# WHU-USI3DV/GAGS

Measured on AMD Instinct MI355X. Metric: feature-raster fwd+bwd views/s, higher is better.
Workload: dtype f32

## Files before the change

### gags_amd/_lib.py

```python
import ctypes
import os
import subprocess

import torch

_HERE = os.path.dirname(os.path.abspath(__file__))
CSRC = os.path.join(_HERE, "csrc")
LIB_PATH = os.path.join(CSRC, "libgags_hip.so")

_vp, _i32, _i64, _f32, _f64 = ctypes.c_void_p, ctypes.c_int, ctypes.c_int64, ctypes.c_float, ctypes.c_double

SIGNATURES = {
    "gags_abi_version": (_i32, []),
    "gags_strerror": (ctypes.c_char_p, [_i32]),
    "gags_device_count": (_i32, []),
    "gags_project_fwd": (_i32, [_i32, _vp, _vp, _vp, _vp, _vp, _i32, _i32, _f32, _f32, _f32, _f32,
                                _vp, _vp, _vp, _vp, _vp, _vp]),
    "gags_project_fwd_raw": (_i32, [_i32, _vp, _vp, _vp, _vp, _f32, _vp, _vp, _i32, _i32, _f32, _f32, _f32, _f32,
                                    _vp, _vp, _vp, _vp, _vp, _vp, _vp, _vp, _vp, _vp]),
    "gags_project_bwd_raw": (_i32, [_i32, _vp, _vp, _vp, _vp, _f32, _vp, _vp, _i32, _i32, _f32, _vp, _vp, _vp, _vp, _vp,
                                    _vp, _vp, _vp, _vp, _vp]),
    "gags_scan_scratch_bytes": (_i64, [_i32]),
    "gags_cumsum_i32": (_i32, [_i32, _vp, _vp, _vp, _vp, _i64, _vp]),
    "gags_cumsum_gather_i32": (_i32, [_i32, _vp, _vp, _vp, _vp, _vp, _i64, _vp]),
# ... 55 lines not shown
    "gags_sam_clip_feature": (_i32, [_i32, _i32, _i32, _i32, _i32, _i32, _vp, _vp, _vp, _vp, _vp, _vp]),
    "gags_sam_clip_feature_bwd_scale": (_i32, [_i32, _i32, _i32, _i32, _i32, _i32, _vp, _vp, _vp, _vp, _vp]),
    "gags_distill_l1_map_fwd": (_i32, [_i32, _i32, _i32, _i32, _i32, _i32, _vp, _vp, _vp, _vp, _vp, _vp, _i32, _vp]),
    "gags_distill_l1_map_bwd": (_i32, [_i32, _i32, _i32, _i32, _i32, _i32, _vp, _vp, _vp, _vp, _vp, _vp, _vp, _i32, _vp]),
    "gags_decoder_head_distill_fwd": (_i32, [_i32, _i32, _i32, _i32, _i32, _i32, _i32, _vp, _vp, _vp, _vp, _vp, _vp, _vp]),
    "gags_decoder_head_distill_bwd": (_i32, [_i32, _i32, _i32, _i32, _i32, _i32, _i32, _vp, _vp, _vp, _vp, _vp, _vp, _vp, _vp]),
    "gags_decoder_head_distill_bwd_f32": (_i32, [_i32, _i32, _i32, _i32, _i32, _i32, _i32, _vp, _vp, _vp, _vp, _vp, _vp, _vp, _vp]),
    "gags_decoder_pack_input": (_i32, [_i64, _i32, _i32, _vp, _vp, _vp]),
    "gags_decoder_pack_layer": (_i32, [_i32, _i32, _vp, _vp, _vp, _vp, _vp, _vp, _vp, _vp]),
    "gags_decoder_pack_layers": (_i32, [_i32, _vp, _vp, _vp, _vp, _vp, _vp, _vp, _vp, _vp, _vp]),
    "gags_decoder_layer": (_i32, [_i64, _i32, _i32, _vp, _vp, _vp, _vp, _i32, _vp, _vp, _vp, _vp, _vp, _vp]),
    "gags_decoder_wgrad_scratch_bytes": (_i64, [_i64, _i32, _i32]),
    "gags_decoder_wgrad": (_i32, [_i64, _i32, _i32, _vp, _vp, _vp, _vp, _vp, _vp, _i64, _vp]),
    "gags_decoder_wgrad_out": (_i32, [_i64, _i32, _i32, _vp, _vp, _vp, _vp, _vp, _i32, _i32, _vp, _vp, _i64, _vp]),
    "gags_decoder_head_bwd": (_i32, [_i64, _i32, _i32, _i32, _vp, _vp, _vp, _i32, _vp]),
    "gags_decoder_unpack_grad": (_i32, [_i64, _i32, _i32, _vp, _vp, _vp]),
    "gags_decoder_head": (_i32, [_i64, _i32, _i32, _i32, _vp, _vp, _i32, _vp]),
    "gags_decoder_fwd_fused": (_i32, [_i64, _i32, _i32, _vp, _vp, _vp, _vp, _vp, _vp, _vp]),
    "gags_decoder_bwd_fused": (_i32, [_i64, _i32, _i32, _vp, _vp, _vp, _vp, _vp, _vp]),
    "gags_decoder_bwd_fused_scaled": (_i32, [_i64, _i32, _i32, _vp, _vp, _vp, _vp, _vp, _vp, _vp]),
    "gags_scale_decoder_fwd_fused": (_i32, [_i64, _i32, _vp, _vp, _vp, _vp, _vp, _vp, _vp]),
    "gags_scale_decoder_fwd_fused_head": (_i32, [_i64, _i32, _vp, _vp, _vp, _vp, _vp, _vp, _vp, _vp]),
    "gags_softmax_head_bwd_y": (_i32, [_i64, _i32, _i32, _vp, _vp, _vp, _vp]),
    "gags_scale_decoder_bwd_fused": (_i32, [_i64, _vp, _vp, _vp, _vp, _vp]),
    "gags_decoder_layer_exact": (_i32, [_i64, _i32, _i32, _vp, _vp, _i32, _vp, _vp, _i32, _vp, _vp, _vp, _vp, _i32, _vp]),
    "gags_decoder_layer_split": (_i32, [_i64, _i32, _i32, _vp, _vp, _i32, _vp, _vp, _i32, _vp, _vp, _vp, _vp, _i32, _i32, _vp]),
    "gags_decoder_wgrad_split": (_i32, [_i64, _i32, _i32, _vp, _i32, _vp, _vp, _i32, _vp, _vp, _vp, _i64, _i32, _vp]),
    "gags_decoder_wgrad_exact_scratch_bytes": (_i64, [_i64, _i32, _i32]),
    "gags_decoder_wgrad_exact": (_i32, [_i64, _i32, _i32, _vp, _i32, _vp, _vp, _i32, _vp, _vp, _vp, _i64, _vp]),
    "gags_decoder_head_bwd_exact": (_i32, [_i64, _i32, _i32, _i32, _vp, _vp, _i32, _vp, _i32, _vp]),
    **{name + "_h16": None for name in ("gags_decoder_pack_layer", "gags_decoder_pack_layers", "gags_decoder_pack_input", "gags_decoder_layer", "gags_decoder_head",
                                        "gags_decoder_wgrad_scratch_bytes", "gags_decoder_wgrad", "gags_decoder_wgrad_out",
                                        "gags_decoder_head_bwd",
                                        "gags_decoder_unpack_grad", "gags_decoder_fwd_fused", "gags_decoder_bwd_fused", "gags_decoder_bwd_fused_scaled",
                                        "gags_scale_decoder_fwd_fused", "gags_scale_decoder_bwd_fused", "gags_scale_decoder_fwd_fused_head",
                                        "gags_softmax_head_bwd_y")},
    "gags_pow2_scale": (_i32, [_vp, _f32, _f32, _vp, _vp]),
    "gags_decoder_head_distill_bwd_h16": (_i32, [_i32, _i32, _i32, _i32, _i32, _i32, _i32, _vp, _vp, _vp, _vp, _vp, _vp, _vp, _vp, _vp]),
    "gags_relevancy": (_i32, [_i64, _i32, _i32, _i32, _vp, _vp, _vp, _vp, _vp]),
    "gags_relevancy_activate_scratch_bytes": (_i64, [_i32, _i32, _i32]),
    "gags_relevancy_activate": (_i32, [_i32, _i32, _i32, _vp, _f32, _i32, _i32, _vp, _vp, _vp, _vp, _vp, _vp, _vp, _i64, _vp]),
    "gags_point_relevancy_mask_scratch_bytes": (_i64, [_i32, _i64]),
    "gags_point_relevancy_mask": (_i32, [_i32, _i64, _vp, _f32, _vp, _vp, _vp, _i64, _vp]),
    "gags_point_mask_smooth_scratch_bytes": (_i64, [_i32, _i64]),
    "gags_point_mask_smooth": (_i32, [_i32, _i64, _vp, _vp, _f64, _i32, _vp, _vp, _vp, _i64, _vp]),
    "gags_depthsample_scratch_bytes": (_i64, [_i64, _i32, _i32, _i32]),
    "gags_depthsample_map": (_i32, [_i64, _i32, _i32, _i32, _vp, _vp, _vp, _vp, _f32, _i32, _vp, _vp, _vp, _vp, _i64, _vp]),
    "gags_depthsample_scatter": (_i32, [_i64, _i32, _i32, _i32, _vp, _vp, _vp, _vp, _f32, _i32, _vp, _vp, _vp, _i64, _vp]),
    "gags_photometric_partials": (_i64, [_i32, _i32, _i32]),
    "gags_photometric_fwd": (_i32, [_i32, _i32, _i32, _i32, _vp, _i64, _i64, _i64, _vp, _i64, _i64, _i64, _vp, _f64, _f64, _f64,
                                    _i32, _vp, _vp, _vp, _vp, _vp, _vp, _vp]),
    "gags_photometric_bwd": (_i32, [_i32, _i32, _i32, _i32, _vp, _i64, _i64, _i64, _vp, _i64, _i64, _i64, _vp, _vp, _vp, _vp,
                                    _i64, _i64, _i64, _vp]),
    "gags_densify_stats": (_i32, [_i32, _vp, _vp, _vp, _vp, _f32, _f32, _vp, _vp, _vp, _vp]),
    "gags_densify_decide": (_i32, [_i32, _vp, _vp, _vp, _vp, _f32, _f32, _f32, _f32, _f32, _i32, _vp, _vp]),
    "gags_densify_plan": (_i32, [_i32, _vp, _vp, _vp, _i64, _vp, _vp, _vp, _vp]),
    "gags_densify_gather": (_i32, [_i64, _vp, _vp, _i32, _vp, _vp]),
    "gags_densify_children": (_i32, [_i64, _i64, _i32, _vp, _vp, _vp, _vp, _vp, _vp, _i64, _vp, _vp, _vp]),
    "gags_reset_opacity": (_i32, [_i64, _vp, _vp, _vp, _vp]),
    "gags_knn3_dist2_scratch_bytes": (_i64, [_i64]),
    "gags_knn3_dist2": (_i32, [_i64, _vp, _vp, _vp, _i64, _vp]),
    "gags_masks_max_count": (_i32, []),
    "gags_masks_pair_chunk_words": (_i32, []),
    "gags_masks_pack": (_i32, [_i32, _i64, _vp, _vp, _vp, _vp]),
    "gags_masks_pairs": (_i32, [_i32, _i64, _vp, _vp, _vp]),
    "gags_masks_colmax": (_i32, [_i32, _vp, _vp, _vp, _vp, _vp]),
    "gags_masks_paint": (_i32, [_i32, _i64, _vp, _i32, _vp, _i32, _vp, _vp]),
    "gags_masks_nms_scratch_bytes": (_i64, [_i32, _i64]),
    "gags_masks_nms_colmax": (_i32, [_i32, _i64, _vp, _vp, _vp, _vp, _vp, _i64, _vp]),
}

for _name in [k for k, v in SIGNATURES.items() if v is None]:
    SIGNATURES[_name] = SIGNATURES[_name[:-4]]

GAGS_BWD_COLORS_ONLY = 1
GAGS_FWD_NO_MFMA = 2
GAGS_FWD_ONLY_WEIGHTS, GAGS_FWD_ONLY_FEATURES = 512, 1024
GAGS_RECS_BY_GAUSSIAN = 256
GAGS_BWD_ATOMIC = 4
GAGS_FEAT_F16 = 32
GAGS_BWD_F32MFMA = 64
GAGS_BWD_BLOCKWAVES = 4096
GAGS_BWD_EXACT_WEIGHTS = 8192
GAGS_BWD_F16SPLIT = 0
GAGS_FWD_F16MFMA = 128
GAGS_FWD_F16MFMA_C = 64
GAGS_FWD_EXACT = 2048
GAGS_FWD_FUSED = 8
GAGS_STAGE_ALL, GAGS_STAGE_ROWS, GAGS_STAGE_SORT, GAGS_STAGE_REDUCE, GAGS_STAGE_MASK = 0, 1, 2, 3, 15
GAGS_STAGED_F32MFMA, GAGS_STAGED_OUT_F16, GAGS_STAGED_PREZEROED = 32, 64, 128
GAGS_STAGED_RANGE_SCRATCH, GAGS_STAGED_BLOCKWAVES, GAGS_STAGED_EXACT_WEIGHTS = 256, 512, 1024
GAGS_KIND_KEEP, GAGS_KIND_CLONE, GAGS_KIND_CHILD_A, GAGS_KIND_CHILD_B = 0, 1, 2, 3
GAGS_GATHER_MAX_DESC, GAGS_GATHER_COPY, GAGS_GATHER_MOMENT = 24, 0, 1


class GatherDesc(ctypes.Structure):
    _fields_ = [("in_", _vp), ("out", _vp), ("row_floats", ctypes.c_int32), ("mode", ctypes.c_int32)]


GAGS_GEOM_F32MFMA = 32

_lib = None


class GagsLibraryError(RuntimeError):
    pass


def build(verbose=False):
    out = None if verbose else subprocess.DEVNULL
    subprocess.check_call(["make", "-C", CSRC, "-j8", "libgags_hip.so"], stdout=out)
    return LIB_PATH


def load():
    global _lib
    if _lib is not None:
        return _lib
    if not os.path.exists(LIB_PATH):
        raise GagsLibraryError(
            f"{LIB_PATH} is missing: build it with `python -c 'import __graft_entry__ as g; g.build()'` "
            "or `make -C gags_amd/csrc`.  gags_amd has no CPU / PyTorch fallback.")
    try:
        lib = ctypes.CDLL(LIB_PATH)
    except OSError as e:
        raise GagsLibraryError(f"cannot load {LIB_PATH}: {e}") from e
    for name, (res, args) in SIGNATURES.items():
        try:
            fn = getattr(lib, name)
        except AttributeError as e:
            raise GagsLibraryError(f"{LIB_PATH} does not export {name}") from e
        fn.restype = res
        fn.argtypes = args
    _lib = lib
    return lib


def check(code, what):
    if code != 0:
        msg = load().gags_strerror(code)
        raise RuntimeError(f"{what} failed: {msg.decode() if msg else code} ({code})")


def ptr(t):
    return None if t is None else ctypes.c_void_p(t.data_ptr())
```

### gags_amd/csrc/launch.h

```cpp
#pragma once
#include "common.h"

inline int64_t al256(int64_t x) { return (x + 255) / 256 * 256; }

struct GagsTiles {
    int w, h, n;
};
inline GagsTiles gags_tiles(int width, int height)
{
    const int w = (width + GAGS_TILE - 1) / GAGS_TILE, h = (height + GAGS_TILE - 1) / GAGS_TILE;
    return {w, h, w * h};
}

constexpr int GAGS_MAX_DEVICES = 16;
template <int N>
inline bool gags_raise_dynamic_lds(bool (&raised)[GAGS_MAX_DEVICES], const void *const (&kernels)[N], int bytes)
{
    int dev = 0;
    if (hipGetDevice(&dev) != hipSuccess || dev < 0) return false;
    if (dev < GAGS_MAX_DEVICES && raised[dev]) return true;
    for (const void *k : kernels)
        if (hipFuncSetAttribute(k, hipFuncAttributeMaxDynamicSharedMemorySize, bytes) != hipSuccess) return false;
    if (dev < GAGS_MAX_DEVICES) raised[dev] = true;
    return true;
}

int64_t gags_sort_u32_scratch_bytes(int64_t n);
int gags_sort_pairs_u32(int64_t n, int nbits, const uint32_t *keys_in, const int32_t *vals_in, uint32_t *keys_out,
                        int32_t *vals_out, void *scratch, int64_t scratch_bytes, hipStream_t st);
int64_t gags_sort_u64_scratch_bytes(int64_t n);
int gags_sort_pairs_u64(int64_t n, int first_bit, int nbits, const uint64_t *keys_in, const int32_t *vals_in,
                        uint64_t *keys_out, int32_t *vals_out, void *scratch, int64_t scratch_bytes, hipStream_t st);

int gags_raster_fwd_valu(int d, int width, int height, const float *means2d, const float *conics,
                         const float *opacities, const float *colors, const float *backgrounds,
                         const int32_t *offsets, const int32_t *flat, int n_isects, float *out, float *alphas,
                         int32_t *last_ids, hipStream_t st);
int gags_raster_bwd_valu(int d, int width, int height, const float *means2d, const float *conics,
                         const float *opacities, const float *colors, const float *backgrounds,
                         const int32_t *offsets, const int32_t *flat, int n_isects, const float *alphas,
                         const int32_t *last_ids, const float *v_out, const float *v_alpha, float *v_colors,
                         float *v_opac, float *v_m2d, float *v_con, bool geom, hipStream_t st);

int gags_pack_isects_launch(int n, int n_isects, const int32_t *flat, const float *means2d, const float *conics,
                            const float *opacities, const int32_t *radii, void *grec, void *packed, hipStream_t st);
int gags_raster_weights_launch(int width, int height, int n_gauss, const void *packed, int by_gauss, const int32_t *offsets,
                               const int32_t *flat, int n_isects, float *wt, int32_t *gid_s, int32_t *sidx_s,
                               int32_t *hit, int32_t *blk_rows, float *Tbuf, float *alphas, int32_t *last_ids,
                               hipStream_t st, const float *colors16 = nullptr, const float *backgrounds = nullptr,
                               float *render_colors = nullptr);
int gags_list_need_launch(int width, int height, int n_gauss, const void *packed, int by_gauss, const int32_t *offsets,
                          const int32_t *flat, int n_isects, int32_t *need, hipStream_t st);
int gags_trim_offsets_launch(int n_tiles, const int32_t *cum, int32_t *off_new, hipStream_t st);
int gags_trim_gather_launch(int n_tiles, const int32_t *off_old, const int32_t *off_new, const int32_t *flat_in, int32_t *flat_out,
                            hipStream_t st);
int gags_trim_last_ids_launch(int width, int height, const int32_t *off_old, const int32_t *off_new, const float *alphas,
                              int32_t *last_ids, hipStream_t st);

int gags_raster_fwd_feat_launch(int d, int width, int height, int n_gauss, const float *colors, int colors_f16, int exact,
                                const float *backgrounds, const int32_t *offsets, int n_isects,
                                const int32_t *blk_rows, const float *wt, const int32_t *gid_s, const float *Tbuf,
                                float *out, hipStream_t st);
int gags_raster_fwd_fused_launch(int d, int width, int height, const void *packed, const float *colors,
                                 const float *backgrounds, const int32_t *offsets, const int32_t *flat, int n_isects,
                                 float *out, float *alphas, int32_t *last_ids, int by_gauss, hipStream_t st);

int64_t gags_bwd_staged_scratch_bytes_impl(int64_t rows, int n_gauss, int d);
int gags_raster_bwd_staged_launch(int d, int width, int height, int n_gauss, const int32_t *offsets, int n_isects,
                                  const float *v_out, const int32_t *blk_rows, const int32_t *trow, int64_t rows,
                                  const float *wt, const int32_t *gid_s, const int32_t *trow_s, void *scratch,
                                  int64_t scratch_bytes, float *v_colors, int stage_flags, int ch_begin, int ch_count,
                                  const int32_t *rows_dev, const int32_t *wire_pos, float *wire, const uint8_t *keep_prev,
                                  uint8_t *keep_cur, hipStream_t st);
int gags_bwd_slot_rows_launch(int width, int height, int n_isects, const int32_t *offsets, const int32_t *blk_rows,
                              const int32_t *sidx_s, const int32_t *trow, int32_t *trow_s, hipStream_t st);

int gags_rows_group_launch(int64_t rows, int n_gauss, const int32_t *rows_dev, uint32_t *key, int32_t *idx, uint32_t *key_s,
                           int32_t *idx_s, int32_t *seg, void *sort_scratch, int64_t sort_scratch_bytes, hipStream_t st);
int gags_rows_reduce_launch(int n_gauss, int d, int ch_begin, int ch_count, const int32_t *seg, const int32_t *idx_s,
                            const float *prow, int pitch, void *out, bool out_f16, hipStream_t st, int sparse = 0,
                            const int32_t *wire_pos = nullptr, float *wire = nullptr, const uint8_t *keep_prev = nullptr,
                            uint8_t *keep_cur = nullptr);

int64_t gags_raster_bwd_geom_scratch_bytes_impl(int64_t n_isects, int width, int height, int n_gauss, int d, int64_t n_rows);
int gags_raster_bwd_geom_launch(int d, int n_gauss, int width, int height, const float *colors, const float *backgrounds,
                                const int32_t *offsets, int n_isects, const void *packed, const float *v_out,
                                const float *v_alphas, const int32_t *blk_rows, const float *wt, const int32_t *gid_s,
                                const int32_t *sidx_s, const float *Tbuf, void *scratch, int64_t scratch_bytes, float *v_geo,
                                int by_gauss, const int32_t *row_base, int64_t n_rows, const int32_t *hit,
                                const int32_t *flatten_ids, int f32mfma, hipStream_t st);
int gags_blended_mask_launch(int n_isects, const int32_t *hit, const int32_t *flatten_ids, unsigned char *mask, hipStream_t st);

int gags_raster_bwd_atomic_launch(int d, int width, int height, const void *packed, const int32_t *offsets,
                                  const int32_t *flat, int n_isects, const float *v_out, float *v_colors,
                                  int by_gauss, hipStream_t st);
```

### gags_amd/csrc/raster_bwd_rows.hip

```cpp
#include <cstdlib>
#include "raster_mfma_common.h"
#include "launch.h"

using namespace gags_mfma;

namespace {

constexpr int CMAX = 64;

template <int NBR>
__global__ __launch_bounds__(256, (NBR == 4 ? 2 : (NBR == 2 ? 3 : 4))) void raster_bwd_rows(
    int d, int width, int height, int tile_w, int n_tiles, int ch_base, int n_slices,
    const float *__restrict__ v_render_colors, const int32_t *__restrict__ offsets, int n_isects,
    const int32_t *__restrict__ blk_rows, const int32_t *__restrict__ trow, const float *__restrict__ wt,
    const int32_t *__restrict__ gid_s, const int32_t *__restrict__ trow_s, float *__restrict__ prow, int prow_pitch,
    uint32_t *__restrict__ row_key, int32_t *__restrict__ row_idx, int rows_cap)
{
    constexpr int CW = 32 * NBR;
    constexpr int C4 = CW / 4;
    __shared__ __attribute__((aligned(16))) float stage[4][32][CW];
    __shared__ __attribute__((aligned(4))) uint8_t pos[2][CMAX][4];
    __shared__ int cand[2][4];
    __shared__ __attribute__((aligned(16))) float zrow[CW];

// ... 401 lines not shown
    L.seg = o; o += al256(((int64_t)n_gauss + 2) * 4);
    L.sort = o; o += al256(gags_sort_u32_scratch_bytes(rows));
    L.prow = o; o += al256(rows * (int64_t)d * 4);
    L.total = o;
    return L;
}

}

int64_t gags_bwd_staged_scratch_bytes_impl(int64_t rows, int n_gauss, int d)
{
    return staged_layout(rows > 0 ? rows : 1, n_gauss, d).total;
}

int gags_bwd_slot_rows_launch(int width, int height, int n_isects, const int32_t *offsets, const int32_t *blk_rows,
                              const int32_t *sidx_s, const int32_t *trow, int32_t *trow_s, hipStream_t st)
{
    GAGS_CLEAR_ERR();
    const int n_tiles = gags_tiles(width, height).n;
    hipLaunchKernelGGL(slot_rows_kernel, dim3(n_tiles * GAGS_BLOCKS_PER_TILE), dim3(64), 0, st, n_tiles, n_isects, offsets, blk_rows, sidx_s, trow, trow_s);
    GAGS_CHECK_LAUNCH();
    return GAGS_OK;
}

static bool rows_scale_per_block()
{
    static const bool v = [] { const char *e = getenv("GAGS_BWD_ROWSCALE"); return e && e[0] == '1'; }();
    return v;
}

int gags_raster_bwd_staged_launch(int d, int width, int height, int n_gauss, const int32_t *offsets, int n_isects,
                                  const float *v_out, const int32_t *blk_rows, const int32_t *trow, int64_t rows,
                                  const float *wt, const int32_t *gid_s, const int32_t *trow_s, void *scratch,
                                  int64_t scratch_bytes, float *v_colors, int stage_flags, int ch_begin, int ch_count,
                                  const int32_t *rows_dev, const int32_t *wire_pos, float *wire, const uint8_t *keep_prev,
                                  uint8_t *keep_cur, hipStream_t st)
{
    GAGS_CLEAR_ERR();
    const int stage = stage_flags & GAGS_STAGE_MASK;
    if (!gags_mfma_width(d) || d > 1024) return 1;
    const bool sA = stage == GAGS_STAGE_ALL || stage == GAGS_STAGE_ROWS, sS = stage == GAGS_STAGE_ALL || stage == GAGS_STAGE_SORT,
               sR = stage == GAGS_STAGE_ALL || stage == GAGS_STAGE_REDUCE;
    const GagsTiles T = gags_tiles(width, height);
    if (ch_count <= 0 || ch_begin < 0 || ch_begin + ch_count > d || ch_begin % 32 != 0 ||
        (ch_count % 32 != 0 && ch_begin + ch_count != d))
        return GAGS_EINVAL;
    const bool narrow = (stage_flags & GAGS_STAGED_RANGE_SCRATCH) != 0;
    const int pp = narrow ? ((ch_count + 3) & ~3) : d;
    const StagedLayout L = staged_layout(rows > 0 ? rows : 1, n_gauss, pp);
    if (scratch_bytes < L.total) return GAGS_ESCRATCH;
    char *sb = (char *)scratch;
    uint32_t *key = (uint32_t *)(sb + L.key), *key_s = (uint32_t *)(sb + L.key_s);
    int32_t *idx = (int32_t *)(sb + L.idx), *idx_s = (int32_t *)(sb + L.idx_s), *seg = (int32_t *)(sb + L.seg);
    float *prow = (float *)(sb + L.prow) - (narrow ? ch_begin : 0);
    if (rows > 0 && sA) {
#define GAGS_ROWS_LAUNCH(KERNEL, CH0, NSL)                                                                           \
    hipLaunchKernelGGL(KERNEL, dim3(T.n * (NSL)), dim3(256), 0, st, d, width, height, T.w, T.n, (CH0), (NSL),           \
                       v_out, offsets, n_isects, blk_rows, trow, wt, gid_s, trow_s, prow, pp, key, idx, (int)rows)
        int c = ch_begin;
        const int ce = ch_begin + ch_count;
        if (ce - c >= 128) {
            const int nsl = (ce - c) / 128;
            if (stage_flags & GAGS_STAGED_F32MFMA) GAGS_ROWS_LAUNCH(raster_bwd_rows<4>, c, nsl);
            else if (stage_flags & GAGS_STAGED_BLOCKWAVES) GAGS_ROWS_LAUNCH(raster_bwd_rows_f16, c, nsl);
            else if (stage_flags & GAGS_STAGED_EXACT_WEIGHTS) GAGS_ROWS_LAUNCH((raster_bwd_rows_cw<3, 5>), c, nsl);
            else if (rows_scale_per_block()) GAGS_ROWS_LAUNCH((raster_bwd_rows_cw<2, 3>), c, nsl);
            else GAGS_ROWS_LAUNCH((raster_bwd_rows_cw<2, 3, true>), c, nsl);
            c += 128 * nsl;
        }
        if (ce - c >= 64) {
            GAGS_ROWS_LAUNCH(raster_bwd_rows<2>, c, 1);
            c += 64;
        }
        if (ce - c > 0) GAGS_ROWS_LAUNCH(raster_bwd_rows<1>, c, (ce - c + 31) / 32);
#undef GAGS_ROWS_LAUNCH
    }
    if (sS) {
        const int rc = gags_rows_group_launch(rows, n_gauss, rows_dev, key, idx, key_s, idx_s, seg, sb + L.sort, L.prow - L.sort, st);
        if (rc != GAGS_OK) return rc;
    }
    if (sR) {
        const bool half = (stage_flags & GAGS_STAGED_OUT_F16) != 0;
        const int sparse = (stage_flags & GAGS_STAGED_PREZEROED) ? 1 : 0;
        const int rc = gags_rows_reduce_launch(n_gauss, d, ch_begin, ch_count, seg, idx_s, prow, pp, v_colors, half, st, sparse, wire_pos,
                                               wire, keep_prev, keep_cur);
        if (rc != GAGS_OK) return rc;
    }
    GAGS_CHECK_LAUNCH();
    return GAGS_OK;
}
```

### gags_amd/csrc/rows_reduce.hip

```cpp
#include <hip/hip_fp16.h>
#include "launch.h"

namespace {

__global__ __launch_bounds__(256) void row_tail_kernel(int64_t cap, const int32_t *__restrict__ total, int n_gauss,
                                                       uint32_t *__restrict__ row_key, int32_t *__restrict__ row_idx)
{
    const int64_t i = (int64_t)blockIdx.x * 256 + threadIdx.x;
    if (i >= cap || i < (int64_t)total[0]) return;
    row_key[i] = (uint32_t)n_gauss;
    row_idx[i] = 0;
}

__global__ __launch_bounds__(256) void seg_offsets_kernel(int n, const uint32_t *__restrict__ sorted_keys, int n_keys,
                                                          int32_t *__restrict__ seg)
{
    const int i = blockIdx.x * 256 + threadIdx.x;
    if (i >= n) return;
    const int cur = min((int)sorted_keys[i], n_keys);
    if (i == 0) {
        for (int g = 0; g <= cur; ++g) seg[g] = 0;
    } else {
        const int prev = min((int)sorted_keys[i - 1], n_keys);
        for (int g = prev + 1; g <= cur; ++g) seg[g] = i;
    }
    if (i == n - 1)
        for (int g = cur + 1; g <= n_keys; ++g) seg[g] = n;
}

__global__ void seg_fill_kernel(int n_keys, int32_t *__restrict__ seg)
{
    const int g = blockIdx.x * 256 + threadIdx.x;
    if (g <= n_keys) seg[g] = 0;
}

constexpr int REDUCE_ITER = 8;
template <bool HALF, int VW>
__global__ __launch_bounds__(256) void reduce_rows_kernel(int n_gauss, int d, int ch_begin, int ch_count,
                                                          const int32_t *__restrict__ seg,
                                                          const int32_t *__restrict__ sorted_rows,
                                                          const float *__restrict__ prow, int prow_pitch,
                                                          void *__restrict__ v_colors_, int sparse,
                                                          const int32_t *__restrict__ wire_pos, float *__restrict__ wire,
                                                          const uint8_t *__restrict__ keep_prev, uint8_t *__restrict__ keep_cur,
                                                          int tail)
{
    const int lpg = ch_count / VW;
    const int gpb = 256 / lpg;
    const int gl = threadIdx.x / lpg;
    const int cl = ch_begin + (threadIdx.x % lpg) * VW;
    if (gl >= gpb) return;
    for (int it = 0; it < REDUCE_ITER; ++it) {
    const int g = (blockIdx.x * REDUCE_ITER + it) * gpb + gl;
    if (g >= n_gauss) return;
        const int b = seg[g], e = seg[g + 1];
        const bool has = b != e;
        bool write_grad = sparse ? has : true;
        const bool on_wire = wire && wire_pos[g] >= 0;
        if (keep_cur) {
            if (threadIdx.x % lpg == 0) keep_cur[g] = (has || on_wire) ? 1 : 0;
            write_grad = has || keep_prev[g] != 0;
        }
        if (!write_grad && !on_wire) continue;
        const bool skip_grad = !write_grad;
        if constexpr (VW == 1) {
            float acc = 0.f;
            for (int i = b; i < e; ++i) acc += prow[(size_t)sorted_rows[i] * prow_pitch + cl];
            if (!skip_grad) {
                if constexpr (HALF) reinterpret_cast<__half *>(v_colors_)[(size_t)g * d + cl] = __float2half_rn(acc);
                else reinterpret_cast<float *>(v_colors_)[(size_t)g * d + cl] = acc;
            }
            if (wire) {
                const int q = wire_pos[g];
                if (q >= 0) wire[(size_t)q * ch_count + (cl - ch_begin)] = acc;
            }
        } else {
            float4 acc = make_float4(0.f, 0.f, 0.f, 0.f);
            const int tl = threadIdx.x % lpg;
            const bool has_tail = tl < tail;
            const int ct = ch_begin + ch_count + (has_tail ? tl : 0);
            float acc_t = 0.f;
            for (int i = b; i < e; i += 8) {
                int r[8];
#pragma unroll
                for (int j = 0; j < 8; ++j) r[j] = sorted_rows[min(i + j, e - 1)];
                float4 v[8];
                float vt[8];
#pragma unroll
                for (int j = 0; j < 8; ++j) {
                    v[j] = *reinterpret_cast<const float4 *>(prow + (size_t)r[j] * prow_pitch + cl);
                    vt[j] = has_tail ? prow[(size_t)r[j] * prow_pitch + ct] : 0.f;
                }
#pragma unroll
                for (int j = 0; j < 8; ++j) {
                    if (i + j < e) {
                        acc.x += v[j].x; acc.y += v[j].y; acc.z += v[j].z; acc.w += v[j].w;
                        acc_t += vt[j];
                    }
                }
            }
            if (!skip_grad && has_tail) {
                if constexpr (HALF) reinterpret_cast<__half *>(v_colors_)[(size_t)g * d + ct] = __float2half_rn(acc_t);
                else reinterpret_cast<float *>(v_colors_)[(size_t)g * d + ct] = acc_t;
            }
            if (!skip_grad) {
                if constexpr (HALF) {
                    const __half2 lo = __floats2half2_rn(acc.x, acc.y), hi = __floats2half2_rn(acc.z, acc.w);
                    uint2 w;
                    w.x = *reinterpret_cast<const unsigned *>(&lo);
                    w.y = *reinterpret_cast<const unsigned *>(&hi);
                    *reinterpret_cast<uint2 *>(reinterpret_cast<__half *>(v_colors_) + (size_t)g * d + cl) = w;
                } else {
                    typedef float nt_f4 __attribute__((ext_vector_type(4)));
                    __builtin_nontemporal_store(nt_f4{acc.x, acc.y, acc.z, acc.w},
                                                reinterpret_cast<nt_f4 *>(reinterpret_cast<float *>(v_colors_) + (size_t)g * d + cl));
                }
            }
            if (wire) {
                const int q = wire_pos[g];
                if (q >= 0) *reinterpret_cast<float4 *>(wire + (size_t)q * ch_count + (cl - ch_begin)) = acc;
            }
        }
    }
}

}

int gags_rows_group_launch(int64_t rows, int n_gauss, const int32_t *rows_dev, uint32_t *key, int32_t *idx, uint32_t *key_s,
                           int32_t *idx_s, int32_t *seg, void *sort_scratch, int64_t sort_scratch_bytes, hipStream_t st)
{
    if (rows <= 0) {
        hipLaunchKernelGGL(seg_fill_kernel, dim3((n_gauss + 1 + 255) / 256), dim3(256), 0, st, n_gauss, seg);
        return GAGS_OK;
    }
    const dim3 grid((unsigned)((rows + 255) / 256));
    if (rows_dev) hipLaunchKernelGGL(row_tail_kernel, grid, dim3(256), 0, st, rows, rows_dev, n_gauss, key, idx);
    int nbits = 1;
    while ((1ll << nbits) <= n_gauss) ++nbits;
    const int rc = gags_sort_pairs_u32(rows, nbits, key, idx, key_s, idx_s, sort_scratch, sort_scratch_bytes, st);
    if (rc != GAGS_OK) return rc;
    hipLaunchKernelGGL(seg_offsets_kernel, grid, dim3(256), 0, st, (int)rows, key_s, n_gauss, seg);
    return GAGS_OK;
}

int gags_rows_reduce_launch(int n_gauss, int d, int ch_begin, int ch_count, const int32_t *seg, const int32_t *idx_s,
                            const float *prow, int pitch, void *out, bool out_f16, hipStream_t st, int sparse,
                            const int32_t *wire_pos, float *wire, const uint8_t *keep_prev, uint8_t *keep_cur)
{
    const int c4 = ch_count & ~3, c1 = ch_count & 3;
    if (wire && (c1 != 0 || !wire_pos)) return GAGS_EINVAL;
    const bool ride = c4 >= 16 && c1 > 0;
    auto reduce = [&](auto *k_f16, auto *k_f32, int vw, int c0, int cw, int tail) {
        const int gpb = 256 / (cw / vw);
        const dim3 grid((n_gauss + gpb * REDUCE_ITER - 1) / (gpb * REDUCE_ITER));
        hipLaunchKernelGGL(out_f16 ? k_f16 : k_f32, grid, dim3(256), 0, st, n_gauss, d, c0, cw, seg, idx_s, prow, pitch, out, sparse,
                           wire_pos, wire, keep_prev, keep_cur, tail);
    };
    if (c4 > 0) reduce((reduce_rows_kernel<true, 4>), (reduce_rows_kernel<false, 4>), 4, ch_begin, c4, ride ? c1 : 0);
    if (c1 > 0 && !ride) reduce((reduce_rows_kernel<true, 1>), (reduce_rows_kernel<false, 1>), 1, ch_begin + c4, c1, 0);
    return GAGS_OK;
}
```

### gags_amd/rasterization.py

```python
import ctypes
import os
import threading
from typing import Any, NamedTuple

import torch

from . import _lib, profiler
from ._lib import check, ptr

TILE = 16
MAX_ISECTS = 1 << 28
ZERO_FILL_MIN_ELEMS = 1 << 24
GEOM_COMPACT_ROWS = True
CAP_MARGIN = 1.05
GRAD_RANGE_CHANNELS = 128
GRAD_ROWS_GROUP = 128
PROW_MAX_BYTES = 24 << 30
TRIM_LISTS = {"1": True, "0": False}.get(os.environ.get("GAGS_TRIM_LISTS", ""), None)
TRIM_AUTO_BYTES = 48 << 30
KEEP_GRAD = os.environ.get("GAGS_KEEP_GRAD", "1") != "0"
KEEP_GRAD_MIN_ELEMS = 0
KEEP_GRAD_SHAPES = 2
EARLY_COUNT = os.environ.get("GAGS_EARLY_COUNT", "1") != "0"
EARLY_ROWMAP = os.environ.get("GAGS_EARLY_ROWMAP", "1") != "0"
# ... 566 lines not shown
    v_geo = torch.empty(fwd.n, 8, device=dev)
    with profiler.stage("raster_bwd_geom"):
        check(lib.gags_raster_bwd_geom(fwd.d, fwd.n, fwd.width, fwd.height, ptr(colors), ptr(backgrounds), ptr(fwd.offsets),
                                       fwd.n_isects, ptr(packed), ptr(v_out), ptr(v_alphas), ptr(fwd.blk_rows),
                                       ptr(fwd.fwd_scratch), fwd.fwd_scratch.numel(), ptr(gscratch), nb, ptr(v_geo),
                                       ptr(fwd.flatten_ids), ptr(row_base), n_rows, _geom_flags(route), _stream()),
              "gags_raster_bwd_geom")
    return v_geo[:, 3:5].contiguous(), v_geo[:, 0:3].contiguous(), v_colors, v_geo[:, 5].contiguous()


def _backward_valu(lib, route, fwd, means2d, conics, opacities, colors, backgrounds, packed, alphas, last_ids, v_out, v_alphas):
    dev = colors.device
    if route.half:
        colors = colors.float()
    v_colors = torch.zeros(fwd.n, fwd.d, device=dev)
    v_opac, v_m2d, v_con = ([torch.zeros(fwd.n, *k, device=dev) for k in ((), (2,), (3,))] if route.geom else (None, None, None))
    with profiler.stage("raster_bwd"):
        check(lib.gags_raster_bwd(fwd.d, fwd.width, fwd.height, ptr(means2d), ptr(conics), ptr(opacities), ptr(colors),
                                  ptr(backgrounds), ptr(fwd.offsets), ptr(fwd.flatten_ids), fwd.n_isects, ptr(packed),
                                  ptr(alphas), ptr(last_ids), ptr(v_out), ptr(v_alphas), ptr(v_colors),
                                  ptr(v_opac), ptr(v_m2d), ptr(v_con), _bwd_flags(route), _stream()), "gags_raster_bwd")
    return v_m2d, v_con, v_colors.half() if route.half else v_colors, v_opac


def _channel_ranges(d, spec):
    if isinstance(spec, int):
        if spec <= 0 or d % spec != 0 or d <= spec or spec % 32 != 0:
            return None
        return [(c, c + spec) for c in range(0, d, spec)]
    widths = [int(w) for w in spec]
    if not widths or any(w <= 0 or w % 128 != 0 for w in widths) or d % 128 != 0 or d <= widths[0]:
        return None
    out, c, i = [], 0, 0
    while c < d:
        w = min(widths[min(i, len(widths) - 1)], d - c)
        out.append((c, c + w))
        c, i = c + w, i + 1
    return out


class _EarlyRowmap:

    def __init__(self, trow, total, stmp, host, ev, rctx, dev):
        self.trow, self.total, self.stmp, self.host, self.ev, self.rctx, self.dev = trow, total, stmp, host, ev, rctx, dev
        self._rows = None

    def rows(self):
        if self._rows is None:
            self.ev.synchronize()
            self._rows = int(self.host[0])
            self.rctx.give_pinned(self.dev, self.host)
            self.host = None
        return self._rows

    def __del__(self):
        try:
            if self.host is not None:
                if self.ev.query():
                    self.rctx.give_pinned(self.dev, self.host)
                self.host = None
        except Exception:
            pass


class _FwdState(NamedTuple):
    offsets: Any
    n_isects: int
    blk_rows: Any
    fwd_scratch: Any
    flatten_ids: Any
    n: int
    d: int
    width: int
    height: int


_STAGE_NAMES = {_lib.GAGS_STAGE_ROWS: "bwd_rows", _lib.GAGS_STAGE_SORT: "bwd_sort", _lib.GAGS_STAGE_REDUCE: "bwd_reduce"}


def _stage_bits(raster_flags, half):
    return ((_lib.GAGS_STAGED_F32MFMA if (raster_flags & _lib.GAGS_BWD_F32MFMA) else 0)
            | (_lib.GAGS_STAGED_OUT_F16 if half else 0)
            | (_lib.GAGS_STAGED_BLOCKWAVES if (raster_flags & _lib.GAGS_BWD_BLOCKWAVES) else 0)
            | (_lib.GAGS_STAGED_EXACT_WEIGHTS if (raster_flags & _lib.GAGS_BWD_EXACT_WEIGHTS) else 0))


_C_SHARED = _lib.GAGS_BWD_COLORS_ONLY | _lib.GAGS_FWD_NO_MFMA


def _fwd_flags(route):
    return ((route.flags & (_C_SHARED | _lib.GAGS_FWD_EXACT)) | _lib.GAGS_RECS_BY_GAUSSIAN
            | (_lib.GAGS_FEAT_F16 if route.half else 0)
            | (_lib.GAGS_FWD_F16MFMA_C if (route.half and route.flags & _lib.GAGS_FWD_F16MFMA) else 0))


def _bwd_flags(route):
    return (route.flags & _C_SHARED) | _lib.GAGS_RECS_BY_GAUSSIAN | (0 if route.geom else _lib.GAGS_BWD_COLORS_ONLY)


def _geom_flags(route):
    return _lib.GAGS_RECS_BY_GAUSSIAN | (_lib.GAGS_GEOM_F32MFMA if (route.flags & _lib.GAGS_BWD_F32MFMA) else 0)


def _rowmap(lib, fwd):
    dev = fwd.blk_rows.device
    ne = lib.gags_bwd_rowmap_elems(fwd.n_isects, fwd.width, fwd.height)
    trow = torch.empty(ne, dtype=torch.int32, device=dev)
    total = torch.empty(1, dtype=torch.int32, device=dev)
    sb = lib.gags_bwd_rowmap_scratch_bytes(fwd.n_isects)
    stmp = torch.empty(max(sb, 4), dtype=torch.uint8, device=dev)
    check(lib.gags_bwd_rowmap(fwd.n_isects, fwd.width, fwd.height, ptr(fwd.offsets), ptr(fwd.blk_rows), ptr(fwd.fwd_scratch),
                              fwd.fwd_scratch.numel(), ptr(trow), ne, ptr(total), ptr(stmp), sb, _stream()), "gags_bwd_rowmap")
    return trow, total, stmp


def _early_rowmap(lib, rctx, fwd):
    trow, total, stmp = _rowmap(lib, fwd)
    dev = total.device
    host = rctx.take_pinned(dev)
    host.copy_(total, non_blocking=True)
    ev = torch.cuda.Event()
    ev.record()
    return _EarlyRowmap(trow, total, stmp, host, ev, rctx, dev)


def _row_count(lib, rctx, fwd, early, capacity):
    if early is not None:
        return early.trow, early.total, early.rows(), None
    with profiler.stage("bwd_rowcount"):
        trow, total, _ = _rowmap(lib, fwd)
        if capacity is not None:
            return trow, total, min(max(fwd.n_isects, 1), int(capacity * CAP_MARGIN) + 1024), _DeferredCount(total, rctx)
        host = ctypes.c_int32(0)
        check(lib.gags_read_i32(ptr(total), ctypes.byref(host), _stream()), "gags_read_i32")
        return trow, total, int(host.value), None


def _grad_buffer(rctx, fwd, bits, dev, hook, wire_hook, pending, prezero):
    v_dtype = torch.float16 if (bits & _lib.GAGS_STAGED_OUT_F16) else torch.float32
    if prezero is not None:
        buf, ev = prezero
        if hook is None and buf.shape == (fwd.n, fwd.d) and buf.dtype == v_dtype:
            torch.cuda.current_stream().wait_event(ev)
            return buf, None, bits | _lib.GAGS_STAGED_PREZEROED
    elif pending is None and (hook is None or (wire_hook is not None and rctx.grad_rows_hook is not None)):
        kept = rctx.kept_grad(fwd.n, fwd.d, v_dtype, dev)
        if kept is not None:
            return kept[0], kept, bits
    return torch.empty(fwd.n, fwd.d, device=dev, dtype=v_dtype), None, bits


def _bind_staged(lib, fwd, v_out, trow, rows, scratch, v_colors):
    fixed = (fwd.d, fwd.n, fwd.width, fwd.height, ptr(fwd.offsets), fwd.n_isects, ptr(v_out), ptr(fwd.blk_rows), ptr(trow), rows,
             ptr(fwd.fwd_scratch), fwd.fwd_scratch.numel(), ptr(scratch), scratch.numel(), ptr(v_colors))
    st = _stream()
    with_reduce = (_lib.GAGS_STAGE_ALL, _lib.GAGS_STAGE_REDUCE)

    def call(stage, c0, cw, rows_dev=None, wire=None, keep=None):
        if keep is not None and (stage & _lib.GAGS_STAGE_MASK) not in with_reduce:
            keep = None
        check(lib.gags_raster_bwd_colors_staged(
            *fixed, stage, c0, cw, rows_dev, ptr(wire[0]) if wire else None, ptr(wire[1]) if wire else None,
            ptr(keep[1]) if keep else None, ptr(keep[2]) if keep else None, st), "gags_raster_bwd_colors_staged")

    return call


# ... 231 lines not shown
```

### include/gags_raster.h

```cpp
#ifndef GAGS_RASTER_H
#define GAGS_RASTER_H

#include <stdint.h>

#ifdef __cplusplus
extern "C" {
#endif
#pragma GCC visibility push(default)

#define GAGS_TILE 16
#define GAGS_MAX_ISECTS (1ll << 28)

#define GAGS_OK 0
#define GAGS_EINVAL (-1)
#define GAGS_ELAUNCH (-2)
#define GAGS_ESCRATCH (-3)
#define GAGS_ENODEV (-4)

#define GAGS_BWD_COLORS_ONLY 1
#define GAGS_FWD_NO_MFMA 2
#define GAGS_FEAT_F16 32
#define GAGS_FWD_F16MFMA 64

#define GAGS_FWD_EXACT 2048
// ... 20 lines not shown
int gags_cumsum_gather_i32(int n, const int32_t *in, const int32_t *idx, int32_t *cum, int32_t *total,
                           void *scratch, int64_t scratch_bytes, void *stream);

int gags_read_i32(const int32_t *src, int32_t *dst_host, void *stream);

int64_t gags_depth_order_scratch_bytes(int n);
int gags_depth_order(int n, const float *depths, const int32_t *tiles_per_gauss, int32_t *order,
                     int32_t *tiles_ordered, void *scratch, int64_t scratch_bytes, void *stream);

int gags_tile_emit(int n, const float *means2d, const int32_t *radii, const float *depths,
                   const int32_t *cum, const int32_t *order, int tile_w, int tile_h,
                   int64_t *isect_ids, int32_t *flatten_ids, void *stream);

int gags_tile_emit_cap(int n, const float *means2d, const int32_t *radii, const float *depths, const int32_t *cum,
                       const int32_t *order, int tile_w, int tile_h, int64_t *isect_ids, int32_t *flatten_ids, int64_t cap,
                       const int32_t *total, void *stream);

int64_t gags_sort_scratch_bytes(int64_t n_isects);
int gags_sort_pairs(int64_t n_isects, int tile_bits, int depth_sorted,
                    const int64_t *keys_in, const int32_t *vals_in,
                    int64_t *keys_out, int32_t *vals_out,
                    void *scratch, int64_t scratch_bytes, void *stream);

int gags_tile_offsets(int64_t n_isects, const int64_t *sorted_ids, int n_tiles,
                      int32_t *isect_offsets, void *stream);

#define GAGS_PACKED_BYTES 32
int gags_pack_isects(int n, int64_t n_isects, const int32_t *flatten_ids, const float *means2d,
                     const float *conics, const float *opacities, const int32_t *radii, void *grec,
                     void *packed, void *stream);

int64_t gags_raster_fwd_scratch_bytes(int64_t n_isects, int width, int height);
int gags_raster_fwd(int d, int n, int width, int height, const float *means2d, const float *conics,
                    const float *opacities, const float *colors, const float *backgrounds,
                    const int32_t *isect_offsets, const int32_t *flatten_ids, int64_t n_isects,
                    const void *packed ,
                    float *render_colors, float *render_alphas, int32_t *last_ids,
                    void *scratch, int64_t scratch_bytes, int32_t *blk_rows,
                    int flags, void *stream);

int gags_raster_list_need(int n, int width, int height, const int32_t *isect_offsets, const int32_t *flatten_ids,
                          int64_t n_isects, const void *packed, int flags, int32_t *need, void *stream);
int gags_trim_lists(int width, int height, const int32_t *isect_offsets, const int32_t *need_cum,
                    const int32_t *flatten_ids, int32_t *offsets_out, int32_t *flatten_out, void *stream);
int gags_trim_last_ids(int width, int height, const int32_t *isect_offsets, const int32_t *offsets_trimmed,
                       const float *render_alphas, int32_t *last_ids, void *stream);

int gags_raster_bwd(int d, int width, int height, const float *means2d, const float *conics,
                    const float *opacities, const float *colors, const float *backgrounds,
                    const int32_t *isect_offsets, const int32_t *flatten_ids, int64_t n_isects,
                    const void *packed ,
                    const float *render_alphas, const int32_t *last_ids,
                    const float *v_render_colors, const float *v_render_alphas,
                    float *v_colors, float *v_opacities, float *v_means2d, float *v_conics,
                    int flags, void *stream);

int64_t gags_bwd_rowmap_elems(int64_t n_isects, int width, int height);
int64_t gags_bwd_rowmap_scratch_bytes(int64_t n_isects);
int gags_bwd_rowmap(int64_t n_isects, int width, int height, const int32_t *isect_offsets, const int32_t *blk_rows,
                    const void *fwd_scratch, int64_t fwd_scratch_bytes, int32_t *rowmap, int64_t rowmap_elems,
                    int32_t *total, void *scratch, int64_t scratch_bytes, void *stream);
#define GAGS_GEOM_F32MFMA 32
int64_t gags_raster_bwd_geom_scratch_bytes(int64_t n_isects, int width, int height, int n, int d, int64_t n_rows);
int gags_raster_bwd_geom(int d, int n, int width, int height, const float *colors, const float *backgrounds,
                         const int32_t *isect_offsets, int64_t n_isects, const void *packed,
                         const float *v_render_colors, const float *v_render_alphas, const int32_t *blk_rows,
                         const void *fwd_scratch, int64_t fwd_scratch_bytes, void *scratch, int64_t scratch_bytes,
                         float *v_geo, const int32_t *flatten_ids, const int32_t *row_base, int64_t n_rows, int flags,
                         void *stream);

int gags_blended_mask(int64_t n_isects, int width, int height, int n, const int32_t *flatten_ids,
                      const void *fwd_scratch, int64_t fwd_scratch_bytes, unsigned char *mask, void *stream);
#define GAGS_STAGE_ALL 0
#define GAGS_STAGE_ROWS 1
#define GAGS_STAGE_SORT 2
#define GAGS_STAGE_REDUCE 3
#define GAGS_STAGE_MASK 15
#define GAGS_STAGED_F32MFMA 32
#define GAGS_STAGED_OUT_F16 64
#define GAGS_STAGED_PREZEROED 128
#define GAGS_STAGED_RANGE_SCRATCH 256
#define GAGS_STAGED_BLOCKWAVES 512
#define GAGS_STAGED_EXACT_WEIGHTS 1024
int64_t gags_bwd_staged_scratch_bytes(int64_t rows, int n, int d);
int gags_raster_bwd_colors_staged(int d, int n, int width, int height, const int32_t *isect_offsets, int64_t n_isects,
                                  const float *v_render_colors, const int32_t *blk_rows, const int32_t *rowmap, int64_t rows,
                                  const void *fwd_scratch, int64_t fwd_scratch_bytes, void *scratch, int64_t scratch_bytes,
                                  float *v_colors, int stage, int ch_begin, int ch_count, const int32_t *rows_dev,
                                  const int32_t *wire_pos, float *wire, const uint8_t *keep_prev, uint8_t *keep_cur,
                                  void *stream);

int gags_raster_stats(int width, int height, const float *means2d, const float *conics,
                      const float *opacities, const int32_t *isect_offsets, const int32_t *flatten_ids,
                      int64_t n_isects, int64_t *counts, void *stream);

int gags_project_fwd_raw(int n, const float *means, const float *rotation, const float *scaling_log,
                         const float *opacity_logit, float scaling_modifier, const float *viewmat, const float *K,
                         int width, int height, float eps2d, float near_plane, float far_plane, float radius_clip,
                         int32_t *radii, float *means2d, float *depths, float *conics, int32_t *tiles_per_gauss,
                         float *opacities, float *quats_act, float *scales_act, void *grec, void *stream);
int gags_project_bwd_raw(int n, const float *means, const float *rotation, const float *scaling_log,
                         const float *opacity_logit, float scaling_modifier, const float *viewmat, const float *K,
                         int width, int height, float eps2d, const int32_t *radii, const float *v_means2d,
                         const float *v_depths, const float *v_conics, const float *v_opacities, float *v_means,
                         float *v_rotation, float *v_scaling_log, float *v_opacity_logit, void *stream);

int gags_project_bwd(int n, const float *means, const float *quats, const float *scales,
                     const float *viewmat, const float *K, int width, int height, float eps2d,
                     const int32_t *radii, const float *conics,
                     const float *v_means2d, const float *v_depths, const float *v_conics,
                     float *v_means, float *v_quats, float *v_scales, void *stream);

int gags_sh_fwd(int n, int kc, int degree, const float *means, const float *campos,
                const float *coeffs, const int32_t *radii, float *out, void *stream);
int gags_sh_bwd(int n, int kc, int degree, const float *means, const float *campos,
                const int32_t *radii, const float *colors_out, const float *v_out,
                float *v_coeffs, void *stream);

int gags_sh_bwd_dirs(int n, int kc, int degree, const float *means, const float *campos, const float *coeffs,
                     const int32_t *radii, const float *colors_out, const float *v_out, float *v_means, void *stream);

int gags_ed_normalize(int64_t n_pix, int d, float *render_colors, const float *render_alphas,
                      void *stream);

int gags_adam_step(int64_t numel, float *param, const float *grad, float *exp_avg, float *exp_avg_sq,
                   double lr, double beta1, double beta2, double eps, int step, void *stream);

int64_t gags_compact_mask_scratch_bytes(int n);
int gags_compact_mask(int n, const uint8_t *mask, int64_t cap, int64_t *idx, int32_t *count, void *scratch,
                      int64_t scratch_bytes, void *stream);
int gags_compact_mask_pos(int n, const uint8_t *mask, int64_t cap, int64_t *idx, int32_t *pos, int32_t *count, void *scratch,
                          int64_t scratch_bytes, void *stream);
int gags_pack_rows(int64_t n_rows, const int64_t *idx, const void *grad, int grad_type, int d, int c0, int cw,
                   void *wire, int wire_type, void *stream);
int gags_unpack_rows(int64_t n_rows, const int64_t *idx, const void *wire, int wire_type, const void *local,
                     void *grad, int grad_type, int d, int c0, int cw, void *stream);

int64_t gags_dot_scratch_bytes(void);
int gags_dot_f32(int64_t numel, const float *x, const float *y, float *out, void *scratch,
                 int64_t scratch_bytes, void *stream);

#pragma GCC visibility pop
#ifdef __cplusplus
}
#endif
#endif
```

Before: 132.3.

## Add row-chunked segmented walk reduction for staged color-gradient reduce

New measurement: 131.6. About the same (-0.5%).

```diff
diff --git a/gags_amd/_lib.py b/gags_amd/_lib.py
--- a/gags_amd/_lib.py
+++ b/gags_amd/_lib.py
@@ -161,6 +161,7 @@
 GAGS_BWD_F32MFMA = 64
 GAGS_BWD_BLOCKWAVES = 4096
 GAGS_BWD_EXACT_WEIGHTS = 8192
+GAGS_BWD_REDUCE_BY_GAUSSIAN = 16384
 GAGS_BWD_F16SPLIT = 0
 GAGS_FWD_F16MFMA = 128
 GAGS_FWD_F16MFMA_C = 64
@@ -169,6 +170,7 @@
 GAGS_STAGE_ALL, GAGS_STAGE_ROWS, GAGS_STAGE_SORT, GAGS_STAGE_REDUCE, GAGS_STAGE_MASK = 0, 1, 2, 3, 15
 GAGS_STAGED_F32MFMA, GAGS_STAGED_OUT_F16, GAGS_STAGED_PREZEROED = 32, 64, 128
 GAGS_STAGED_RANGE_SCRATCH, GAGS_STAGED_BLOCKWAVES, GAGS_STAGED_EXACT_WEIGHTS = 256, 512, 1024
+GAGS_STAGED_REDUCE_BY_GAUSSIAN = 2048
 GAGS_KIND_KEEP, GAGS_KIND_CLONE, GAGS_KIND_CHILD_A, GAGS_KIND_CHILD_B = 0, 1, 2, 3
 GAGS_GATHER_MAX_DESC, GAGS_GATHER_COPY, GAGS_GATHER_MOMENT = 24, 0, 1
 
diff --git a/gags_amd/csrc/launch.h b/gags_amd/csrc/launch.h
--- a/gags_amd/csrc/launch.h
+++ b/gags_amd/csrc/launch.h
@@ -80,7 +80,8 @@
 int gags_rows_reduce_launch(int n_gauss, int d, int ch_begin, int ch_count, const int32_t *seg, const int32_t *idx_s,
                             const float *prow, int pitch, void *out, bool out_f16, hipStream_t st, int sparse = 0,
                             const int32_t *wire_pos = nullptr, float *wire = nullptr, const uint8_t *keep_prev = nullptr,
-                            uint8_t *keep_cur = nullptr);
+                            uint8_t *keep_cur = nullptr, const uint32_t *key_s = nullptr, int64_t rows = 0,
+                            bool by_gaussian = false);
 
 int64_t gags_raster_bwd_geom_scratch_bytes_impl(int64_t n_isects, int width, int height, int n_gauss, int d, int64_t n_rows);
 int gags_raster_bwd_geom_launch(int d, int n_gauss, int width, int height, const float *colors, const float *backgrounds,
diff --git a/gags_amd/csrc/raster_bwd_rows.hip b/gags_amd/csrc/raster_bwd_rows.hip
--- a/gags_amd/csrc/raster_bwd_rows.hip
+++ b/gags_amd/csrc/raster_bwd_rows.hip
@@ -507,8 +507,9 @@
     if (sR) {
         const bool half = (stage_flags & GAGS_STAGED_OUT_F16) != 0;
         const int sparse = (stage_flags & GAGS_STAGED_PREZEROED) ? 1 : 0;
+        const bool by_gaussian = (stage_flags & GAGS_STAGED_REDUCE_BY_GAUSSIAN) != 0;
         const int rc = gags_rows_reduce_launch(n_gauss, d, ch_begin, ch_count, seg, idx_s, prow, pp, v_colors, half, st, sparse, wire_pos,
-                                               wire, keep_prev, keep_cur);
+                                               wire, keep_prev, keep_cur, key_s, rows, by_gaussian);
         if (rc != GAGS_OK) return rc;
     }
     GAGS_CHECK_LAUNCH();
diff --git a/gags_amd/csrc/rows_reduce.hip b/gags_amd/csrc/rows_reduce.hip
--- a/gags_amd/csrc/rows_reduce.hip
+++ b/gags_amd/csrc/rows_reduce.hip
@@ -1,4 +1,6 @@
 #include <hip/hip_fp16.h>
+#include <cstdlib>
+#include <type_traits>
 #include "launch.h"
 
 namespace {
@@ -124,6 +126,168 @@
     }
 }
 
+constexpr int WALK_CH = 16;
+constexpr int WALK_MORE = 8;
+constexpr int WAIT_VM0 = 0x0f70;
+template <bool HALF, bool TAIL, int CH>
+__global__ __launch_bounds__(256) void reduce_walk_kernel(int n_rows, int n_gauss, int d, int ch_begin, int c4, int tail,
+                                                          const uint32_t *__restrict__ key_s,
+                                                          const int32_t *__restrict__ idx_s,
+                                                          const float *__restrict__ prow, int prow_pitch,
+                                                          void *__restrict__ v_colors_,
+                                                          const int32_t *__restrict__ wire_pos, float *__restrict__ wire,
+                                                          uint8_t *__restrict__ keep_cur)
+{
+    static_assert(CH + 2 <= 64, "a chunk's keys sit in the lanes of one wave");
+    const int tl = threadIdx.x, lane = threadIdx.x & 63;
+    const bool active = tl < c4 / 4;
+    const int cl = ch_begin + 4 * (active ? tl : 0);
+    const bool has_tail = TAIL && tl < tail;
+    const int ct = ch_begin + c4 + (has_tail ? tl : 0);
+    const int base = blockIdx.x * CH, last = n_rows - 1;
+
+    const int p = base - 1 + lane;
+    uint32_t kv = 0xffffffffu;
+    int rv = 0;
+    if (lane <= CH + 1) {
+        rv = idx_s[min(max(p, 0), last)];
+        if (p >= 0) kv = key_s[min(p, last)];
+    }
+    const uint32_t k_before = __shfl_up(kv, 1), k_after = __shfl_down(kv, 1);
+    const bool live = lane >= 1 && lane <= CH && p <= last && kv < (uint32_t)n_gauss;
+    const unsigned long long start_m = __ballot(live && kv != k_before) >> 1;
+    const unsigned long long cont_m = __ballot(live && p < last && k_after == kv) >> 1;
+    if (!start_m) return;
+    const unsigned long long own_m = (__ballot(live) >> 1) & ~((start_m & (0 - start_m)) - 1);
+    int wq = -1;
+    if (wire && live) wq = wire_pos[kv];
+
+    float4 v[CH];
+    float vt[CH];
+#pragma unroll
+    for (int j = 0; j < CH; ++j) {
+        vt[j] = 0.f;
+        if ((own_m >> j) & 1) {
+            const float *src = prow + (size_t)__builtin_amdgcn_readlane(rv, j + 1) * prow_pitch;
+            if (active) v[j] = *reinterpret_cast<const float4 *>(src + cl);
+            if (has_tail) vt[j] = src[ct];
+        }
+    }
+
+    float zero = 0.f;
+    asm volatile("" : "+v"(zero) : : "memory");
+    __builtin_amdgcn_s_waitcnt(WAIT_VM0);
+    float4 acc = make_float4(zero, zero, zero, zero);
+    float acc_t = zero;
+#pragma unroll
+    for (int j = 0; j < CH; ++j) {
+        if (!((own_m >> j) & 1)) continue;
+        if ((start_m >> j) & 1) {
+            acc = make_float4(zero, zero, zero, zero);
+            acc_t = zero;
+        }
+        acc.x += v[j].x; acc.y += v[j].y; acc.z += v[j].z; acc.w += v[j].w;
+        if constexpr (TAIL) acc_t += vt[j];
+        if ((cont_m >> j) & 1) {
+            if (j < CH - 1) continue;
+        }
+        const uint32_t g = (uint32_t)__builtin_amdgcn_readlane((int)kv, j + 1);
+        if (j == CH - 1 && ((cont_m >> j) & 1)) {
+            for (int pos = base + CH;; pos += WALK_MORE) {
+                uint32_t kk = 0xffffffffu;
+                int rr = 0;
+                if (lane < WALK_MORE && pos + lane <= last) {
+                    rr = idx_s[pos + lane];
+                    kk = key_s[pos + lane];
+                }
+                const unsigned long long same = __ballot(kk == g);
+                const int cnt = __ffsll((long long)~same) - 1;
+                float4 u[WALK_MORE];
+                float ut[WALK_MORE];
+#pragma unroll
+                for (int t = 0; t < WALK_MORE; ++t) {
+                    ut[t] = 0.f;
+                    if (t < cnt) {
+                        const float *src = prow + (size_t)__builtin_amdgcn_readlane(rr, t) * prow_pitch;
+                        if (active) u[t] = *reinterpret_cast<const float4 *>(src + cl);
+                        if (has_tail) ut[t] = src[ct];
+                    }
+                }
+                __builtin_amdgcn_s_waitcnt(WAIT_VM0);
+#pragma unroll
+                for (int t = 0; t < WALK_MORE; ++t) {
+                    if (t < cnt) {
+                        acc.x += u[t].x; acc.y += u[t].y; acc.z += u[t].z; acc.w += u[t].w;
+                        if constexpr (TAIL) acc_t += ut[t];
+                    }
+                }
+                if (cnt < WALK_MORE) break;
+            }
+        }
+        if (has_tail) {
+            if constexpr (HALF) reinterpret_cast<__half *>(v_colors_)[(size_t)g * d + ct] = __float2half_rn(acc_t);
+            else reinterpret_cast<float *>(v_colors_)[(size_t)g * d + ct] = acc_t;
+        }
+        if (active) {
+            if constexpr (HALF) {
+                const __half2 lo = __floats2half2_rn(acc.x, acc.y), hi = __floats2half2_rn(acc.z, acc.w);
+                uint2 w;
+                w.x = *reinterpret_cast<const unsigned *>(&lo);
+                w.y = *reinterpret_cast<const unsigned *>(&hi);
+                *reinterpret_cast<uint2 *>(reinterpret_cast<__half *>(v_colors_) + (size_t)g * d + cl) = w;
+            } else {
+                typedef float nt_f4 __attribute__((ext_vector_type(4)));
+                __builtin_nontemporal_store(nt_f4{acc.x, acc.y, acc.z, acc.w},
+                                            reinterpret_cast<nt_f4 *>(reinterpret_cast<float *>(v_colors_) + (size_t)g * d + cl));
+            }
+        }
+        if (keep_cur && tl == 0) keep_cur[g] = 1;
+        if (wire) {
+            const int q = __builtin_amdgcn_readlane(wq, j + 1);
+            if (q >= 0 && active) *reinterpret_cast<float4 *>(wire + (size_t)q * c4 + 4 * tl) = acc;
+        }
+    }
+}
+
+template <bool HALF>
+__global__ __launch_bounds__(256) void reduce_norows_kernel(int n_gauss, int d, int ch_begin, int ch_count,
+                                                            const int32_t *__restrict__ seg, void *__restrict__ v_colors_,
+                                                            int sparse, const int32_t *__restrict__ wire_pos,
+                                                            float *__restrict__ wire, const uint8_t *__restrict__ keep_prev,
+                                                            uint8_t *__restrict__ keep_cur)
+{
+    const int g = blockIdx.x * 256 + threadIdx.x;
+    const int lane = threadIdx.x & 63;
+    bool zero_grad = false;
+    int q = -1;
+    if (g < n_gauss && seg[g] == seg[g + 1]) {
+        if (wire) q = wire_pos[g];
+        if (keep_cur) {
+            keep_cur[g] = q >= 0 ? 1 : 0;
+            zero_grad = keep_prev[g] != 0;
+        } else {
+            zero_grad = !sparse;
+        }
+    }
+    const int c4 = ch_count & ~3, c1 = ch_count & 3;
+    for (unsigned long long m = __ballot(zero_grad); m; m &= m - 1) {
+        const size_t row = (size_t)(g - lane + (__ffsll((long long)m) - 1)) * d + ch_begin;
+        if constexpr (HALF) {
+            __half *dst = reinterpret_cast<__half *>(v_colors_) + row;
+            for (int c = 4 * lane; c < c4; c += 256) *reinterpret_cast<uint2 *>(dst + c) = make_uint2(0u, 0u);
+            if (lane < c1) dst[c4 + lane] = __float2half_rn(0.f);
+        } else {
+            float *dst = reinterpret_cast<float *>(v_colors_) + row;
+            for (int c = 4 * lane; c < c4; c += 256) *reinterpret_cast<float4 *>(dst + c) = make_float4(0.f, 0.f, 0.f, 0.f);
+            if (lane < c1) dst[c4 + lane] = 0.f;
+        }
+    }
+    for (unsigned long long m = __ballot(q >= 0); m; m &= m - 1) {
+        float *dst = wire + (size_t)__shfl(q, __ffsll((long long)m) - 1) * ch_count;
+        for (int c = 4 * lane; c < c4; c += 256) *reinterpret_cast<float4 *>(dst + c) = make_float4(0.f, 0.f, 0.f, 0.f);
+    }
+}
+
 }
 
 int gags_rows_group_launch(int64_t rows, int n_gauss, const int32_t *rows_dev, uint32_t *key, int32_t *idx, uint32_t *key_s,
@@ -145,10 +309,33 @@
 
 int gags_rows_reduce_launch(int n_gauss, int d, int ch_begin, int ch_count, const int32_t *seg, const int32_t *idx_s,
                             const float *prow, int pitch, void *out, bool out_f16, hipStream_t st, int sparse,
-                            const int32_t *wire_pos, float *wire, const uint8_t *keep_prev, uint8_t *keep_cur)
+                            const int32_t *wire_pos, float *wire, const uint8_t *keep_prev, uint8_t *keep_cur,
+                            const uint32_t *key_s, int64_t rows, bool by_gaussian)
 {
     const int c4 = ch_count & ~3, c1 = ch_count & 3;
     if (wire && (c1 != 0 || !wire_pos)) return GAGS_EINVAL;
+    if (key_s && !by_gaussian && c4 >= 128 && c4 <= 1024 && rows < (int64_t)0x7fffff00) {
+        if (rows > 0) {
+            static const int ch_env = [] { const char *e = getenv("GAGS_REDUCE_CH"); return e ? atoi(e) : WALK_CH; }();
+            auto go = [&](auto chc) {
+                constexpr int CHX = decltype(chc)::value;
+                const dim3 grid((unsigned)((rows + CHX - 1) / CHX)), block((c4 / 4 + 63) / 64 * 64);
+                auto walk = [&](auto *k) {
+                    hipLaunchKernelGGL(k, grid, block, 0, st, (int)rows, n_gauss, d, ch_begin, c4, c1, key_s, idx_s, prow, pitch, out,
+                                       wire_pos, wire, keep_cur);
+                };
+                if (c1 > 0) walk(out_f16 ? reduce_walk_kernel<true, true, CHX> : reduce_walk_kernel<false, true, CHX>);
+                else walk(out_f16 ? reduce_walk_kernel<true, false, CHX> : reduce_walk_kernel<false, false, CHX>);
+            };
+            if (ch_env == 8) go(std::integral_constant<int, 8>{});
+            else if (ch_env == 32) go(std::integral_constant<int, 32>{});
+            else go(std::integral_constant<int, 16>{});
+        }
+        if (!sparse || keep_cur || wire)
+            hipLaunchKernelGGL(out_f16 ? reduce_norows_kernel<true> : reduce_norows_kernel<false>, dim3((n_gauss + 255) / 256),
+                               dim3(256), 0, st, n_gauss, d, ch_begin, ch_count, seg, out, sparse, wire_pos, wire, keep_prev, keep_cur);
+        return GAGS_OK;
+    }
     const bool ride = c4 >= 16 && c1 > 0;
     auto reduce = [&](auto *k_f16, auto *k_f32, int vw, int c0, int cw, int tail) {
         const int gpb = 256 / (cw / vw);
diff --git a/gags_amd/rasterization.py b/gags_amd/rasterization.py
--- a/gags_amd/rasterization.py
+++ b/gags_amd/rasterization.py
@@ -672,7 +672,8 @@
     return ((_lib.GAGS_STAGED_F32MFMA if (raster_flags & _lib.GAGS_BWD_F32MFMA) else 0)
             | (_lib.GAGS_STAGED_OUT_F16 if half else 0)
             | (_lib.GAGS_STAGED_BLOCKWAVES if (raster_flags & _lib.GAGS_BWD_BLOCKWAVES) else 0)
-            | (_lib.GAGS_STAGED_EXACT_WEIGHTS if (raster_flags & _lib.GAGS_BWD_EXACT_WEIGHTS) else 0))
+            | (_lib.GAGS_STAGED_EXACT_WEIGHTS if (raster_flags & _lib.GAGS_BWD_EXACT_WEIGHTS) else 0)
+            | (_lib.GAGS_STAGED_REDUCE_BY_GAUSSIAN if (raster_flags & _lib.GAGS_BWD_REDUCE_BY_GAUSSIAN) else 0))
 
 
 _C_SHARED = _lib.GAGS_BWD_COLORS_ONLY | _lib.GAGS_FWD_NO_MFMA
diff --git a/include/gags_raster.h b/include/gags_raster.h
--- a/include/gags_raster.h
+++ b/include/gags_raster.h
@@ -126,6 +126,7 @@
 #define GAGS_STAGED_RANGE_SCRATCH 256
 #define GAGS_STAGED_BLOCKWAVES 512
 #define GAGS_STAGED_EXACT_WEIGHTS 1024
+enum { GAGS_STAGED_REDUCE_BY_GAUSSIAN = 2048 };
 int64_t gags_bwd_staged_scratch_bytes(int64_t rows, int n, int d);
 int gags_raster_bwd_colors_staged(int d, int n, int width, int height, const int32_t *isect_offsets, int64_t n_isects,
                                   const float *v_render_colors, const int32_t *blk_rows, const int32_t *rowmap, int64_t rows,
```
